# MCG-NJU/MeMOTR

Measured on AMD Instinct MI355X. Metric: train_frames_per_sec, higher is better.
Workload: dtype f32

## Files before the change

### memotr_amd/csrc/clip_attention.h

```cpp
#pragma once

namespace {
constexpr int kLanes = 16;
constexpr int kRows = 256 / kLanes;
constexpr int kHd = 32;
constexpr int kPitch = 36;

__device__ __forceinline__ void load_row32(const float *p, float *r) {
#pragma unroll
    for (int i = 0; i < 8; ++i) {
        const f32x4_t v = *reinterpret_cast<const f32x4_t *>(p + 4 * i);
        r[4 * i] = v.x; r[4 * i + 1] = v.y; r[4 * i + 2] = v.z; r[4 * i + 3] = v.w;
    }
}

__device__ __forceinline__ float dot32(const float *a, const float *lds_row) {
    float s0 = 0.f, s1 = 0.f;
#pragma unroll
    for (int i = 0; i < 8; ++i) {
        const f32x4_t v = *reinterpret_cast<const f32x4_t *>(lds_row + 4 * i);
        s0 = fmaf(a[4 * i], v.x, s0);
        s1 = fmaf(a[4 * i + 1], v.y, s1);
        s0 = fmaf(a[4 * i + 2], v.z, s0);
        s1 = fmaf(a[4 * i + 3], v.w, s1);
    }
    return s0 + s1;
}

__device__ __forceinline__ float dot32r(const float *a, const float *b) {
    float s0 = 0.f, s1 = 0.f;
#pragma unroll
    for (int i = 0; i < 8; ++i) {
        s0 = fmaf(a[4 * i], b[4 * i], s0);
        s1 = fmaf(a[4 * i + 1], b[4 * i + 1], s1);
        s0 = fmaf(a[4 * i + 2], b[4 * i + 2], s0);
        s1 = fmaf(a[4 * i + 3], b[4 * i + 3], s1);
    }
    return s0 + s1;
}

__device__ __forceinline__ void axpy32(float *acc, float w, const float *lds_row) {
#pragma unroll
    for (int i = 0; i < 8; ++i) {
        const f32x4_t v = *reinterpret_cast<const f32x4_t *>(lds_row + 4 * i);
        acc[4 * i] = fmaf(w, v.x, acc[4 * i]);
        acc[4 * i + 1] = fmaf(w, v.y, acc[4 * i + 1]);
        acc[4 * i + 2] = fmaf(w, v.z, acc[4 * i + 2]);
        acc[4 * i + 3] = fmaf(w, v.w, acc[4 * i + 3]);
    }
}

__device__ __forceinline__ float sum8l(float x) {
#pragma unroll
    for (int o = 1; o < kLanes; o <<= 1) x += __shfl_xor(x, o, 64);
    return x;
}
__device__ __forceinline__ float max8l(float x) {
#pragma unroll
    for (int o = 1; o < kLanes; o <<= 1) x = fmaxf(x, __shfl_xor(x, o, 64));
    return x;
}

__device__ __forceinline__ void stage_rows(float *dst, const float *src, long rs, int L) {
    for (int i = threadIdx.x; i < L * 8; i += blockDim.x) {
        const int r = i >> 3, c = (i & 7) * 4;
        *reinterpret_cast<f32x4_t *>(dst + r * kPitch + c) = *reinterpret_cast<const f32x4_t *>(src + r * rs + c);
    }
}

__global__ __launch_bounds__(256) void mha_fwd_kernel(const float *__restrict__ q, const float *__restrict__ k,
                                                     const float *__restrict__ v, long q_bs, long q_rs, long k_bs,
                                                     long k_rs, long v_bs, long v_rs,
                                                     const uint8_t *__restrict__ key_mask, int H, int L, float scale,
                                                     float *__restrict__ out, float *__restrict__ lse) {
    extern __shared__ __attribute__((aligned(16))) float s_mem[];
    float *Ks = s_mem, *Vs = s_mem + (size_t)L * kPitch;
    const int h = blockIdx.y, b = blockIdx.z;
    stage_rows(Ks, k + b * k_bs + h * kHd, k_rs, L);
    stage_rows(Vs, v + b * v_bs + h * kHd, v_rs, L);
    __syncthreads();
    const int row = blockIdx.x * kRows + threadIdx.x / kLanes, sub = threadIdx.x % kLanes;
    const bool row_ok = row < L;
    const int rowc = row_ok ? row : L - 1;
    float qr[kHd];
    load_row32(q + b * q_bs + rowc * q_rs + h * kHd, qr);
#pragma unroll
    for (int i = 0; i < kHd; ++i) qr[i] *= scale;
    const uint8_t *mk = key_mask ? key_mask + (long)b * L : nullptr;
    float m = -INFINITY, l = 0.f, acc[kHd];
#pragma unroll
    for (int i = 0; i < kHd; ++i) acc[i] = 0.f;
    for (int j = sub; j < L; j += kLanes) {
        if (mk && mk[j]) continue;
        const float s = dot32(qr, Ks + j * kPitch);
        const float m_new = fmaxf(m, s);
        const float corr = expf(m - m_new), p = expf(s - m_new);
        l = l * corr + p;
#pragma unroll
        for (int i = 0; i < kHd; ++i) acc[i] *= corr;
        axpy32(acc, p, Vs + j * kPitch);
        m = m_new;
    }
    const float M = max8l(m);
    const float w = (m == -INFINITY) ? 0.f : expf(m - M);
    const float Lsum = sum8l(l * w);
    const float inv = 1.f / Lsum;
    float *o = out + ((long)b * L + rowc) * (H * kHd) + h * kHd;
#pragma unroll
    for (int i = 0; i < kHd; ++i) {
        const float t = sum8l(acc[i] * w) * inv;
        if (row_ok && (i >> 2) == sub) o[i] = t;
    }
    if (row_ok && sub == 0) lse[((long)b * H + h) * L + row] = M + logf(Lsum);
}

__global__ __launch_bounds__(256) void mha_bwd_q_kernel(const float *__restrict__ q, const float *__restrict__ k,
                                                       const float *__restrict__ v, long q_bs, long q_rs, long k_bs,
                                                       long k_rs, long v_bs, long v_rs,
                                                       const uint8_t *__restrict__ key_mask,
                                                       const float *__restrict__ out, const float *__restrict__ lse,
                                                       const float *__restrict__ go, int H, int L, float scale,
                                                       float *__restrict__ gq, long gq_bs, long gq_rs) {
    extern __shared__ __attribute__((aligned(16))) float s_mem[];
    float *Ks = s_mem, *Vs = s_mem + (size_t)L * kPitch;
    const int h = blockIdx.y, b = blockIdx.z;
    stage_rows(Ks, k + b * k_bs + h * kHd, k_rs, L);
    stage_rows(Vs, v + b * v_bs + h * kHd, v_rs, L);
    __syncthreads();
    const int row = blockIdx.x * kRows + threadIdx.x / kLanes, sub = threadIdx.x % kLanes;
    const bool row_ok = row < L;
    const int rowc = row_ok ? row : L - 1;
    float qr[kHd], gr[kHd], acc[kHd];
    load_row32(q + b * q_bs + rowc * q_rs + h * kHd, qr);
    const long orow = ((long)b * L + rowc) * (H * kHd) + h * kHd;
    load_row32(go + orow, gr);
    float D = 0.f;
    {
        float orr[kHd];
        load_row32(out + orow, orr);
        D = dot32r(gr, orr);
    }
#pragma unroll
    for (int i = 0; i < kHd; ++i) { qr[i] *= scale; acc[i] = 0.f; }
    const float ls = lse[((long)b * H + h) * L + rowc];
    const uint8_t *mk = key_mask ? key_mask + (long)b * L : nullptr;
    for (int j = sub; j < L; j += kLanes) {
        if (mk && mk[j]) continue;
        const float p = expf(dot32(qr, Ks + j * kPitch) - ls);
        const float ds = p * (dot32(gr, Vs + j * kPitch) - D);
        axpy32(acc, ds, Ks + j * kPitch);
    }
    float *g = gq + b * gq_bs + rowc * gq_rs + h * kHd;
#pragma unroll
    for (int i = 0; i < kHd; ++i) {
        const float t = sum8l(acc[i]) * scale;
        if (row_ok && (i >> 2) == sub) g[i] = t;
    }
}

__global__ __launch_bounds__(256) void mha_bwd_kv_kernel(const float *__restrict__ q, const float *__restrict__ k,
                                                        const float *__restrict__ v, long q_bs, long q_rs, long k_bs,
                                                        long k_rs, long v_bs, long v_rs,
                                                        const uint8_t *__restrict__ key_mask,
                                                        const float *__restrict__ out, const float *__restrict__ lse,
                                                        const float *__restrict__ go, int H, int L, float scale,
                                                        float *__restrict__ gk, long gk_bs, long gk_rs,
                                                        float *__restrict__ gv, long gv_bs, long gv_rs) {
    extern __shared__ __attribute__((aligned(16))) float s_mem[];
    float *Qs = s_mem, *Gs = s_mem + (size_t)L * kPitch;
    float *s_lse = Gs + (size_t)L * kPitch, *s_D = s_lse + L;
    const int h = blockIdx.y, b = blockIdx.z;
    stage_rows(Qs, q + b * q_bs + h * kHd, q_rs, L);
    for (int i = threadIdx.x; i < L * 8; i += blockDim.x) {
        f32x4_t *p4 = reinterpret_cast<f32x4_t *>(Qs + (i >> 3) * kPitch + (i & 7) * 4);
        *p4 = *p4 * scale;
    }
    stage_rows(Gs, go + (long)b * L * (H * kHd) + h * kHd, (long)H * kHd, L);
    for (int i = threadIdx.x; i < L; i += blockDim.x) s_lse[i] = lse[((long)b * H + h) * L + i];
    __syncthreads();
    for (int i = threadIdx.x; i < L; i += blockDim.x) {
        const float *o = out + ((long)b * L + i) * (H * kHd) + h * kHd;
        float orr[kHd];
        load_row32(o, orr);
        s_D[i] = dot32(orr, Gs + i * kPitch);
    }
    __syncthreads();
    const int row = blockIdx.x * kRows + threadIdx.x / kLanes, sub = threadIdx.x % kLanes;
    const bool row_ok = row < L;
    const int rowc = row_ok ? row : L - 1;
    const bool dead = key_mask && key_mask[(long)b * L + rowc];
    float kr[kHd], vr[kHd], ak[kHd], av[kHd];
    load_row32(k + b * k_bs + rowc * k_rs + h * kHd, kr);
    load_row32(v + b * v_bs + rowc * v_rs + h * kHd, vr);
#pragma unroll
    for (int i = 0; i < kHd; ++i) { ak[i] = 0.f; av[i] = 0.f; }
    if (!dead) {
        for (int i = sub; i < L; i += kLanes) {
            const float p = expf(dot32(kr, Qs + i * kPitch) - s_lse[i]);
            const float ds = p * (dot32(vr, Gs + i * kPitch) - s_D[i]);
            axpy32(av, p, Gs + i * kPitch);
            axpy32(ak, ds, Qs + i * kPitch);
        }
    }
    float *pk = gk + b * gk_bs + rowc * gk_rs + h * kHd, *pv = gv + b * gv_bs + rowc * gv_rs + h * kHd;
#pragma unroll
    for (int i = 0; i < kHd; ++i) {
        const float tk = sum8l(ak[i]), tv = sum8l(av[i]);
        if (row_ok && (i >> 2) == sub) {
            pk[i] = tk;
            pv[i] = tv;
        }
    }
}

std::atomic<unsigned long long> g_lds_fwd{0}, g_lds_bq{0}, g_lds_bkv{0};

int mha_check(const void *q, const void *k, const void *v, int B, int H, int L) {
    if (B < 0 || H <= 0 || L < 0) return fail(1, "clipops_mha: bad dimension");
    if (L > CLIPOPS_MHA_MAX_L) return fail(2, "clipops_mha: L exceeds CLIPOPS_MHA_MAX_L");
    if ((long)B * L > 0 && (!q || !k || !v)) return fail(1, "clipops_mha: null pointer");
    return 0;
}
}

extern "C" {
int clipops_mha_fwd_f32(const float *q, const float *k, const float *v, long q_bs, long q_rs, long k_bs, long k_rs,
                        long v_bs, long v_rs, const uint8_t *key_mask, int B, int H, int L, float scale, float *out,
                        float *lse, void *stream) {
    int rc = mha_check(q, k, v, B, H, L);
    if (rc) return rc;
    if ((long)B * L == 0) return ok();
    if (!out || !lse) return fail(1, "clipops_mha_fwd_f32: null pointer");
    const size_t lds = (size_t)2 * L * kPitch * sizeof(float);
    if ((rc = allow_lds(reinterpret_cast<const void *>(mha_fwd_kernel), lds, g_lds_fwd))) return rc;
    return launch("mha_fwd_kernel", mha_fwd_kernel, dim3((L + kRows - 1) / kRows, H, B), dim3(256), lds, stream, q, k, v,
                  q_bs, q_rs, k_bs, k_rs, v_bs, v_rs, key_mask, H, L, scale, out, lse);
}

int clipops_mha_bwd_f32(const float *q, const float *k, const float *v, long q_bs, long q_rs, long k_bs, long k_rs,
                        long v_bs, long v_rs, const uint8_t *key_mask, const float *out, const float *lse,
                        const float *grad_out, int B, int H, int L, float scale, float *grad_q, long gq_bs, long gq_rs,
                        float *grad_k, long gk_bs, long gk_rs, float *grad_v, long gv_bs, long gv_rs, void *stream) {
    int rc = mha_check(q, k, v, B, H, L);
    if (rc) return rc;
    if ((long)B * L == 0) return ok();
    if (!out || !lse || !grad_out || !grad_q || !grad_k || !grad_v) return fail(1, "clipops_mha_bwd_f32: null pointer");
    const size_t lds_q = (size_t)2 * L * kPitch * sizeof(float);
    const size_t lds_kv = lds_q + (size_t)2 * L * sizeof(float);
    if ((rc = allow_lds(reinterpret_cast<const void *>(mha_bwd_q_kernel), lds_q, g_lds_bq))) return rc;
    if ((rc = allow_lds(reinterpret_cast<const void *>(mha_bwd_kv_kernel), lds_kv, g_lds_bkv))) return rc;
    const dim3 grid((L + kRows - 1) / kRows, H, B);
    if ((rc = launch("mha_bwd_q_kernel", mha_bwd_q_kernel, grid, dim3(256), lds_q, stream, q, k, v, q_bs, q_rs, k_bs, k_rs,
                     v_bs, v_rs, key_mask, out, lse, grad_out, H, L, scale, grad_q, gq_bs, gq_rs)))
        return rc;
    return launch("mha_bwd_kv_kernel", mha_bwd_kv_kernel, grid, dim3(256), lds_kv, stream, q, k, v, q_bs, q_rs, k_bs, k_rs,
                  v_bs, v_rs, key_mask, out, lse, grad_out, H, L, scale, grad_k, gk_bs, gk_rs, grad_v, gv_bs, gv_rs);
}
}
```

### memotr_amd/functions/clip_ops.py

```python
from __future__ import annotations

import ctypes
import os

import torch
import torch.nn.functional as F


def fused(*tensors) -> bool:
    return (os.environ.get("MEMOTR_FUSED_CLIP_OPS", "1") != "0"
            and all(t.is_cuda and (t.dtype == torch.float32 or not t.is_floating_point()) for t in tensors))


def config_key() -> tuple:
    return (os.environ.get("MEMOTR_FUSED_CLIP_OPS", "1"), os.environ.get("MEMOTR_COLSUM_TALL", "1"),
            os.environ.get("MEMOTR_ATTN_KERNELS", "1"), os.environ.get("MEMOTR_FUSED_LN", "1"),
            os.environ.get("MEMOTR_FUSED_SHIFT_RELU", "1"), os.environ.get("MEMOTR_FUSED_LINEAR_BWD", "1"),
            os.environ.get("MEMOTR_FUSED_LINEAR_FWD", "1"), os.environ.get("MEMOTR_LINEAR_STAGED", "1"))


def _lib():
    from .. import _clip_lib
    return _clip_lib


def _stream(t: torch.Tensor) -> int:
    idx = t.device.index
    if idx is not None and idx != torch.cuda.current_device():
        raise RuntimeError(f"clip_ops: tensor on cuda:{idx} but cuda:{torch.cuda.current_device()} is current; "
                           "call torch.cuda.set_device(tensor.device) (one device per process)")
    return torch.cuda.current_stream(t.device).cuda_stream


def _strides3(t: torch.Tensor):
    if t.dim() != 3 or (t.shape[2] > 1 and t.stride(2) != 1):
        raise RuntimeError("expected a (layers, rows, C) tensor with a dense last axis")
    return t.stride(0), t.stride(1)


def match_cost(logits: torch.Tensor, boxes: torch.Tensor, gt_labels: torch.Tensor, gt_boxes: torch.Tensor,
               w_class: float, w_bbox: float, w_giou: float, out: torch.Tensor = None) -> torch.Tensor:
    n_layers, Q, K = logits.shape
    T = gt_labels.shape[0]
    if out is not None:
        assert out.is_contiguous() and out.dtype == torch.float32 and out.numel() == n_layers * Q * T
        cost = out.view(n_layers, Q, T)
    else:
        cost = torch.empty((n_layers, Q, T), dtype=torch.float32, device=logits.device)
    lsl, lsq = _strides3(logits)
    bsl, bsq = _strides3(boxes)
    gt_labels, gt_boxes = gt_labels.contiguous(), gt_boxes.contiguous()
    L = _lib()
    L.check(L.lib.clipops_match_cost_f32(logits.data_ptr(), lsl, lsq, boxes.data_ptr(), bsl, bsq, gt_labels.data_ptr(),
                                         gt_boxes.data_ptr(), n_layers, Q, K, T, float(w_class), float(w_bbox),
                                         float(w_giou), cost.data_ptr(), _stream(logits)), "clipops_match_cost_f32")
    return cost


def track_ownership(track_ids: torch.Tensor, gt_ids: torch.Tensor, free_out: torch.Tensor = None):
    n_tr, n_gt = track_ids.shape[0], gt_ids.shape[0]
    matched = torch.empty((n_tr,), dtype=torch.int64, device=gt_ids.device)
    free = free_out if free_out is not None else torch.empty((n_gt,), dtype=torch.float32, device=gt_ids.device)
    assert free.is_contiguous() and free.dtype == torch.float32 and free.numel() == n_gt
    track_ids, gt_ids = track_ids.contiguous(), gt_ids.contiguous()
    L = _lib()
    L.check(L.lib.clipops_track_ownership_i64(track_ids.data_ptr(), n_tr, gt_ids.data_ptr(), n_gt, matched.data_ptr(),
                                              free.data_ptr(), _stream(gt_ids)), "clipops_track_ownership_i64")
    return matched, free


def track_ownership_reference(track_ids, gt_ids):
    n_gt = gt_ids.shape[0]
    eq = track_ids[:, None] == gt_ids[None, :]
    order = torch.arange(1, n_gt + 1, device=eq.device)
    return (eq * order).amax(1) - 1 if n_gt > 0 else torch.full_like(track_ids, -1), (~eq.any(0)).to(torch.float32)


def focal_labels(lay: torch.Tensor, q: torch.Tensor, g: torch.Tensor, gt_labels: torch.Tensor, matched_idx,
                 late: torch.Tensor, n_det: int, n_tracks: int, num_classes: int) -> torch.Tensor:
    n_layers = late.shape[0]
    labels = torch.empty((n_layers, n_det + n_tracks), dtype=torch.int64, device=late.device)
    lay, q, g, gt_labels = lay.contiguous(), q.contiguous(), g.contiguous(), gt_labels.contiguous()
    L = _lib()
    L.check(L.lib.clipops_focal_labels_i64(lay.data_ptr(), q.data_ptr(), g.data_ptr(), lay.shape[0], gt_labels.data_ptr(),
                                           gt_labels.shape[0], None if matched_idx is None else matched_idx.contiguous().data_ptr(),
                                           n_tracks, late.contiguous().data_ptr(), n_layers, n_det, num_classes,
                                           labels.data_ptr(), _stream(late)), "clipops_focal_labels_i64")
    return labels


def focal_labels_reference(lay, q, g, gt_labels, matched_idx, late, n_det, n_tracks, num_classes):
    n_layers = late.shape[0]
    labels = torch.full((n_layers, n_det + n_tracks), num_classes, dtype=torch.int64, device=late.device)
    labels[lay, q] = gt_labels[g]
    if n_tracks > 0:
        has = matched_idx >= 0
        tr_lab = torch.where(has, gt_labels[matched_idx.clamp(min=0)] if gt_labels.shape[0] > 0
                             else torch.full_like(matched_idx, num_classes), torch.full_like(matched_idx, num_classes))
        labels[:, n_det:] = torch.where(late[:, None], tr_lab[None, :], labels[:, n_det:])
    return labels


class _PairBoxLoss(torch.autograd.Function):
    @staticmethod
    def forward(ctx, boxes_all, lay, qidx, b, tgt_boxes, gidx, weight):
        n_layers, B, Nq, _ = boxes_all.shape
        n = lay.shape[0]
        l1 = torch.empty((n,), dtype=torch.float32, device=boxes_all.device)
        gl = torch.empty_like(l1)
        L = _lib()
        L.check(L.lib.clipops_pair_box_loss_fwd_f32(
            boxes_all.data_ptr(), lay.data_ptr(), qidx.data_ptr(), B * Nq, b * Nq, tgt_boxes.data_ptr(),
            None if gidx is None else gidx.data_ptr(), None if weight is None else weight.data_ptr(), n,
            l1.data_ptr(), gl.data_ptr(), _stream(boxes_all)), "clipops_pair_box_loss_fwd_f32")
        ctx.save_for_backward(boxes_all, lay, qidx, tgt_boxes, gidx, weight)
        ctx.b = b
        return l1, gl

    @staticmethod
    def backward(ctx, g_l1, g_gl):
        boxes_all, lay, qidx, tgt_boxes, gidx, weight = ctx.saved_tensors
        n_layers, B, Nq, _ = boxes_all.shape
        grad = torch.zeros_like(boxes_all)
        L = _lib()
        L.check(L.lib.clipops_pair_box_loss_bwd_f32(
            boxes_all.data_ptr(), lay.data_ptr(), qidx.data_ptr(), B * Nq, ctx.b * Nq, tgt_boxes.data_ptr(),
            None if gidx is None else gidx.data_ptr(), None if weight is None else weight.data_ptr(), lay.shape[0],
            g_l1.contiguous().data_ptr(), g_gl.contiguous().data_ptr(), grad.data_ptr(), _stream(boxes_all)),
            "clipops_pair_box_loss_bwd_f32")
        return grad, None, None, None, None, None, None


def pair_box_loss(boxes_all: torch.Tensor, lay: torch.Tensor, qidx: torch.Tensor, b: int, tgt_boxes: torch.Tensor,
                  gidx: torch.Tensor = None, weight: torch.Tensor = None):
    if not boxes_all.is_contiguous():
        boxes_all = boxes_all.contiguous()
    return _PairBoxLoss.apply(boxes_all, lay.contiguous(), qidx.contiguous(), int(b), tgt_boxes.contiguous(),
                              None if gidx is None else gidx.contiguous(),
                              None if weight is None else weight.contiguous())


def pair_box_loss_reference(boxes_all, lay, qidx, b, tgt_boxes, gidx=None, weight=None):
    from ..models.criterion import paired_giou
    from ..utils.box_ops import box_cxcywh_to_xyxy
    pb = boxes_all[lay, b, qidx]
    tb = tgt_boxes if gidx is None else tgt_boxes[gidx]
    l1 = F.l1_loss(pb, tb, reduction="none").sum(-1)
    gl = 1 - paired_giou(box_cxcywh_to_xyxy(pb), box_cxcywh_to_xyxy(tb))
    if weight is not None:
        l1, gl = l1 * weight, gl * weight
    return l1, gl


def pair_iou(boxes: torch.Tensor, tgt_boxes: torch.Tensor, gidx: torch.Tensor = None) -> torch.Tensor:
    boxes, tgt_boxes = boxes.detach().contiguous(), tgt_boxes.contiguous()
    n = boxes.shape[0]
    out = torch.empty((n,), dtype=torch.float32, device=boxes.device)
    L = _lib()
    L.check(L.lib.clipops_pair_iou_f32(boxes.data_ptr(), tgt_boxes.data_ptr(), None if gidx is None else
                                       gidx.contiguous().data_ptr(), n, out.data_ptr(), _stream(boxes)),
            "clipops_pair_iou_f32")
    return out


def assign(cost: torch.Tensor):
    if cost.dim() != 3 or cost.dtype != torch.float32 or not cost.is_cuda:
        raise RuntimeError("assign expects a float32 CUDA tensor of shape (problems, rows, cols)")
    P, R, C = cost.shape
    k = min(R, C)
    row = torch.empty((P, k), dtype=torch.int32, device=cost.device)
    col = torch.empty((P, k), dtype=torch.int32, device=cost.device)
    status = torch.empty((P,), dtype=torch.int32, device=cost.device)
    L = _lib()
    L.check(L.lib.clipops_assign_f32(cost.data_ptr(), cost.stride(0), cost.stride(1), cost.stride(2), P, R, C,
                                     row.data_ptr(), col.data_ptr(), status.data_ptr(), _stream(cost)),
            "clipops_assign_f32")
    return row, col, status


def pair_iou_reference(boxes, tgt_boxes, gidx=None):
    from ..models.criterion import paired_iou
    from ..utils.box_ops import box_cxcywh_to_xyxy
    tb = tgt_boxes if gidx is None else tgt_boxes[gidx]
    return paired_iou(box_cxcywh_to_xyxy(boxes), box_cxcywh_to_xyxy(tb))


HANDOVER_CARRIED, HANDOVER_NEW, HANDOVER_UNCLAIMED = 0, 1, 2
HANDOVER_DIFF = ("outputs", "queries", "last_ref", "init_ref", "det_embed", "prev_ref", "prev_long", "prev_last",
                 "prev_query")


def handover_tables(n_det: int, n_q: int, n_tracks: int, new_q, new_g, free_q, keep):
    import numpy as np
    n_new, n_free = len(new_q), len(free_q)
    kind = np.concatenate((np.full((n_tracks,), HANDOVER_CARRIED, dtype=np.int64),
                           np.full((n_new,), HANDOVER_NEW, dtype=np.int64),
                           np.full((n_free,), HANDOVER_UNCLAIMED, dtype=np.int64)))
    src = np.concatenate((np.arange(n_tracks, dtype=np.int64), np.asarray(new_q, dtype=np.int64),
                          np.asarray(free_q, dtype=np.int64)))
    gt = np.concatenate((np.full((n_tracks,), -1, dtype=np.int64), np.asarray(new_g, dtype=np.int64),
                         np.full((n_free,), -1, dtype=np.int64)))
    keep = np.asarray(keep, dtype=np.int64)
    table = np.stack((kind[keep], src[keep], gt[keep]), axis=1)
    rows = np.arange(len(keep), dtype=np.int64)
    carried = table[:, 0] == HANDOVER_CARRIED
    inv_q = np.full((n_q,), -1, dtype=np.int64)
    inv_q[np.where(carried, n_det + table[:, 1], table[:, 1])] = rows
    inv_prev = np.full((n_tracks,), -1, dtype=np.int64)
    inv_prev[table[carried, 1]] = rows[carried]
    return np.concatenate((table.reshape(-1), inv_q, inv_prev))


def _handover_views(tables, n_keep, n_q, n_tracks):
    table = tables[:3 * n_keep]
    inv_q = tables[3 * n_keep:3 * n_keep + n_q]
    inv_prev = tables[3 * n_keep + n_q:3 * n_keep + n_q + n_tracks]
    return table, inv_q, inv_prev


def _rows_dense(t):
    return t if t.dim() == 2 and (t.shape[1] == 1 or t.stride(1) == 1) and t.stride(0) >= 0 else t.contiguous()


class _Handover(torch.autograd.Function):
    @staticmethod
    def forward(ctx, outputs, queries, last_ref, init_ref, det_embed, prev_ref, prev_long, prev_last, prev_query,
                logits, boxes, prev_iou, prev_ids, prev_matched, gt_boxes, gt_ids, tables, n_keep, n_det):
        L = _lib()
        use_dab = det_embed is None
        n_q, C, K = outputs.shape[0], outputs.shape[1], logits.shape[1]
        n_tracks, n_gt = prev_ref.shape[0], gt_boxes.shape[0]
        QW = C if use_dab else 2 * C
        named = dict(logits=logits, boxes=boxes, outputs=outputs, queries=queries, last_ref=last_ref, init_ref=init_ref,
                     det_embed=det_embed, prev_ref=prev_ref, prev_long=prev_long, prev_last=prev_last,
                     prev_query=prev_query, prev_iou=prev_iou.reshape(-1, 1))
        widths = dict(logits=K, boxes=4, outputs=C, queries=C, last_ref=4, init_ref=4, det_embed=C, prev_ref=4,
                      prev_long=C, prev_last=C, prev_query=QW, prev_iou=1)
        src, keep = L.HandoverSources(), []
        for i, name in enumerate(L.HANDOVER_SOURCES):
            t = named[name]
            if t is None or t.shape[0] == 0:
                continue
            lead = n_tracks if name.startswith("prev_") else (n_det if name == "det_embed" else n_det + n_tracks)
            if t.dtype != torch.float32 or t.dim() != 2 or t.shape[0] < lead or (
                    t.shape[1] != widths[name] and not (name == "det_embed" and t.shape[1] >= C)):
                raise RuntimeError(f"handover: source {name} has shape {tuple(t.shape)} ({t.dtype})")
            t = _rows_dense(t.detach())
            keep.append(t)
            src.ptr[i], src.row_stride[i] = t.data_ptr(), t.stride(0)
        if n_q != queries.shape[0] or n_q != last_ref.shape[0] or n_q != init_ref.shape[0]:
            raise RuntimeError("handover: the model-output sources differ in their row counts")
        if tables.dtype != torch.int64 or tables.numel() != 3 * n_keep + n_q + n_tracks:
            raise RuntimeError("handover: the table does not have 3 * n_keep + n_q + n_tracks int64 entries")
        tables = tables.contiguous()
        prev_ids, prev_matched, gt_boxes, gt_ids = (t.contiguous() for t in (prev_ids, prev_matched, gt_boxes, gt_ids))
        if n_tracks and (prev_ids.shape[0] != n_tracks or prev_matched.shape[0] != n_tracks):
            raise RuntimeError("handover: ids / matched_idx of the previous set do not have one entry per track")
        dev = outputs.device
        base = torch.empty((n_keep, K + 8 + 3 * C + QW + 1), dtype=torch.float32, device=dev)
        ints = torch.empty((2, n_keep), dtype=torch.int64, device=dev)
        L.check(L.lib.clipops_handover_fwd_f32(
            ctypes.byref(src), prev_ids.data_ptr() if n_tracks else None, prev_matched.data_ptr() if n_tracks else None,
            gt_boxes.data_ptr(), gt_ids.data_ptr(), tables.data_ptr(), n_keep, n_det, n_tracks, n_gt, K, C,
            int(use_dab), base.data_ptr(), ints[0].data_ptr(), ints[1].data_ptr(), _stream(outputs)),
            "clipops_handover_fwd_f32")
        ctx.save_for_backward(tables)
        ctx.dims = (n_keep, n_q, n_det, n_tracks, K, C, use_dab, 0 if det_embed is None else det_embed.shape[1], QW)
        ctx.mark_non_differentiable(ints)
        return base, ints

    @staticmethod
    def backward(ctx, g_base, _g_ints):
        L = _lib()
        (tables,) = ctx.saved_tensors
        n_keep, n_q, n_det, n_tracks, K, C, use_dab, det_cols, QW = ctx.dims
        table, inv_q, inv_prev = _handover_views(tables, n_keep, n_q, n_tracks)
        g_base = g_base.contiguous()
        shapes = dict(outputs=(n_q, C), queries=(n_q, C), last_ref=(n_q, 4), init_ref=(n_q, 4),
                      det_embed=(n_det, det_cols), prev_ref=(n_tracks, 4), prev_long=(n_tracks, C),
                      prev_last=(n_tracks, C), prev_query=(n_tracks, QW))
        wanted = [name for i, name in enumerate(HANDOVER_DIFF) if ctx.needs_input_grad[i]]
        flat = torch.empty((sum(shapes[n][0] * shapes[n][1] for n in wanted),), dtype=torch.float32, device=g_base.device)
        grads, out, pos = L.HandoverGrads(), {}, 0
        for name in wanted:
            r, c = shapes[name]
            out[name] = flat[pos:pos + r * c].view(r, c)
            pos += r * c
            if r * c:
                grads.ptr[L.HANDOVER_SOURCES.index(name)] = out[name].data_ptr()
        if flat.numel():
            L.check(L.lib.clipops_handover_bwd_f32(
                g_base.data_ptr(), table.data_ptr(), inv_q.data_ptr(), inv_prev.data_ptr() if n_tracks else None,
                n_keep, n_q, n_det, n_tracks, K, C, int(use_dab), det_cols, ctypes.byref(grads), _stream(g_base)),
                "clipops_handover_bwd_f32")
        return tuple(out.get(name) for name in HANDOVER_DIFF) + (None,) * 10


def handover(outputs, queries, last_ref, init_ref, det_embed, prev_ref, prev_long, prev_last, prev_query, logits, boxes,
             prev_iou, prev_ids, prev_matched, gt_boxes, gt_ids, tables, n_keep: int, n_det: int):
    base, ints = _Handover.apply(outputs, queries, last_ref, init_ref, det_embed, prev_ref, prev_long, prev_last,
                                 prev_query, logits, boxes, prev_iou, prev_ids, prev_matched, gt_boxes, gt_ids, tables,
                                 n_keep, n_det)
    return base, ints[0], ints[1]


def handover_reference(outputs, queries, last_ref, init_ref, det_embed, prev_ref, prev_long, prev_last, prev_query,
                       logits, boxes, prev_iou, prev_ids, prev_matched, gt_boxes, gt_ids, tables, n_keep: int,
                       n_det: int):
    n_q, C = outputs.shape
    n_tracks = prev_ref.shape[0]
    table, _, _ = _handover_views(tables, n_keep, n_q, n_tracks)
    kind, s, g = table.view(n_keep, 3).unbind(1)
    carried, new = (kind == HANDOVER_CARRIED), (kind == HANDOVER_NEW)
    m = torch.where(carried, n_det + s, s)
    q = torch.where(carried, torch.zeros_like(s), s)

    def prev(t):
        width = 1 if t.dim() == 1 else t.shape[1]
        if n_tracks == 0:
            return t.new_zeros((n_keep, width))
        return t.reshape(n_tracks, width)[torch.where(carried, s, torch.zeros_like(s))]
# ... 742 lines not shown
```

Baseline: 43.67.

## Add v2 fused attention kernels with wider rows, DPP reductions, merged backward

Adds new forward and backward MHA kernels enabled by default via MEMOTR_MHA_V2. The forward kernel uses 512-thread blocks with 32 lanes per query row and caches scores in LDS for a two-pass softmax. It reuses one LDS buffer for K then V (prefetched into registers), skips masked keys, and reduces across lanes with DPP and swizzle. The backward pass merges the dQ and dK/dV kernels into one launch that splits blocks by index and skips dead keys. This cuts launch count and shuffle cost, but adds register pressure and LDS footprint and relies on CLIPOPS_MHA_MAX_L bounds.

```diff
diff --git a/memotr_amd/csrc/clip_attention.h b/memotr_amd/csrc/clip_attention.h
--- a/memotr_amd/csrc/clip_attention.h
+++ b/memotr_amd/csrc/clip_attention.h
@@ -213,7 +213,229 @@
     }
 }
 
-std::atomic<unsigned long long> g_lds_fwd{0}, g_lds_bq{0}, g_lds_bkv{0};
+#define MHA_DPP(x, ctrl) \
+    __builtin_bit_cast(float, __builtin_amdgcn_update_dpp(0, __builtin_bit_cast(int, (x)), (ctrl), 0xF, 0xF, true))
+
+template <int LANES>
+__device__ __forceinline__ float row_sum(float x) {
+    x += MHA_DPP(x, 0xB1);
+    x += MHA_DPP(x, 0x4E);
+    x += MHA_DPP(x, 0x141);
+    x += MHA_DPP(x, 0x140);
+    if (LANES == 32) x += __builtin_bit_cast(float, __builtin_amdgcn_ds_swizzle(__builtin_bit_cast(int, x), 0x401F));
+    return x;
+}
+template <int LANES>
+__device__ __forceinline__ float row_max(float x) {
+    x = fmaxf(x, MHA_DPP(x, 0xB1));
+    x = fmaxf(x, MHA_DPP(x, 0x4E));
+    x = fmaxf(x, MHA_DPP(x, 0x141));
+    x = fmaxf(x, MHA_DPP(x, 0x140));
+    if (LANES == 32) x = fmaxf(x, __builtin_bit_cast(float, __builtin_amdgcn_ds_swizzle(__builtin_bit_cast(int, x), 0x401F)));
+    return x;
+}
+
+constexpr int kLanesW = 32;
+constexpr int kRowsW = 512 / kLanesW;
+constexpr int kRowsQ = 512 / kLanes;
+
+template <int LANES>
+__device__ __forceinline__ unsigned live_keys(const uint8_t *s_mk, int sub, int L) {
+    unsigned live = 0;
+    for (int t = 0; t * LANES < L; ++t) {
+        const int j = sub + t * LANES;
+        const bool on = j < L && !(s_mk && s_mk[min(j, L - 1)]);
+        live |= (unsigned)on << t;
+    }
+    return live;
+}
+
+__host__ __device__ inline size_t mask_bytes(int L) { return (size_t)(L + 15) / 16 * 16; }
+
+__global__ __launch_bounds__(512) void mha2_fwd_kernel(const float *__restrict__ q, const float *__restrict__ k,
+                                                      const float *__restrict__ v, long q_bs, long q_rs, long k_bs,
+                                                      long k_rs, long v_bs, long v_rs,
+                                                      const uint8_t *__restrict__ key_mask, int H, int L, float scale,
+                                                      float *__restrict__ out, float *__restrict__ lse) {
+    constexpr int NV = CLIPOPS_MHA_MAX_L * 8 / 512;
+    extern __shared__ __attribute__((aligned(16))) float s_mem[];
+    const int n_t = (L + kLanesW - 1) / kLanesW;
+    float *s_sc = s_mem + (size_t)L * kPitch + threadIdx.x;
+    uint8_t *s_mk = reinterpret_cast<uint8_t *>(s_mem + (size_t)L * kPitch + (size_t)n_t * 512);
+    const int h = blockIdx.y, b = blockIdx.z;
+    const float *kp = k + b * k_bs + h * kHd, *vp = v + b * v_bs + h * kHd;
+    f32x4_t kreg[NV], vreg[NV];
+#pragma unroll
+    for (int t = 0; t < NV; ++t) {
+        const int i = threadIdx.x + t * 512;
+        if (i < L * 8) kreg[t] = *reinterpret_cast<const f32x4_t *>(kp + (i >> 3) * k_rs + (i & 7) * 4);
+    }
+#pragma unroll
+    for (int t = 0; t < NV; ++t) {
+        const int i = threadIdx.x + t * 512;
+        if (i < L * 8) vreg[t] = *reinterpret_cast<const f32x4_t *>(vp + (i >> 3) * v_rs + (i & 7) * 4);
+    }
+    if (key_mask && (int)threadIdx.x < L) s_mk[threadIdx.x] = key_mask[(long)b * L + threadIdx.x];
+    const int row = blockIdx.x * kRowsW + threadIdx.x / kLanesW, sub = threadIdx.x % kLanesW;
+    const bool row_ok = row < L;
+    const int rowc = row_ok ? row : L - 1;
+    float qr[kHd];
+    load_row32(q + b * q_bs + rowc * q_rs + h * kHd, qr);
+#pragma unroll
+    for (int i = 0; i < kHd; ++i) qr[i] *= scale;
+#pragma unroll
+    for (int t = 0; t < NV; ++t) {
+        const int i = threadIdx.x + t * 512;
+        if (i < L * 8) *reinterpret_cast<f32x4_t *>(s_mem + (i >> 3) * kPitch + (i & 7) * 4) = kreg[t];
+    }
+    __syncthreads();
+    const unsigned live = live_keys<kLanesW>(key_mask ? s_mk : nullptr, sub, L);
+    float m = -INFINITY;
+#pragma unroll 4
+    for (int t = 0; t < n_t; ++t) {
+        const int jc = min(sub + t * kLanesW, L - 1);
+        const float s = (live >> t) & 1u ? dot32(qr, s_mem + jc * kPitch) : -INFINITY;
+        s_sc[t * 512] = s;
+        m = fmaxf(m, s);
+    }
+    const float M = row_max<kLanesW>(m);
+    __syncthreads();
+#pragma unroll
+    for (int t = 0; t < NV; ++t) {
+        const int i = threadIdx.x + t * 512;
+        if (i < L * 8) *reinterpret_cast<f32x4_t *>(s_mem + (i >> 3) * kPitch + (i & 7) * 4) = vreg[t];
+    }
+    __syncthreads();
+    float l = 0.f, acc[kHd];
+#pragma unroll
+    for (int i = 0; i < kHd; ++i) acc[i] = 0.f;
+#pragma unroll 2
+    for (int t = 0; t < n_t; ++t) {
+        const int jc = min(sub + t * kLanesW, L - 1);
+        const float p = (live >> t) & 1u ? expf(s_sc[t * 512] - M) : 0.f;
+        l += p;
+        axpy32(acc, p, s_mem + jc * kPitch);
+    }
+    const float Lsum = row_sum<kLanesW>(l);
+    const float inv = 1.f / Lsum;
+    float *o = out + ((long)b * L + rowc) * (H * kHd) + h * kHd;
+#pragma unroll
+    for (int i = 0; i < kHd; ++i) {
+        const float t = row_sum<kLanesW>(acc[i]) * inv;
+        if (row_ok && (i >> 2) == sub) o[i] = t;
+    }
+    if (row_ok && sub == 0) lse[((long)b * H + h) * L + row] = M + logf(Lsum);
+}
+
+__global__ __launch_bounds__(512) void mha2_bwd_kernel(const float *__restrict__ q, const float *__restrict__ k,
+                                                      const float *__restrict__ v, long q_bs, long q_rs, long k_bs,
+                                                      long k_rs, long v_bs, long v_rs,
+                                                      const uint8_t *__restrict__ key_mask,
+                                                      const float *__restrict__ out, const float *__restrict__ lse,
+                                                      const float *__restrict__ go, int H, int L, float scale,
+                                                      float *__restrict__ gq, long gq_bs, long gq_rs,
+                                                      float *__restrict__ gk, long gk_bs, long gk_rs,
+                                                      float *__restrict__ gv, long gv_bs, long gv_rs, int nblk_q) {
+    extern __shared__ __attribute__((aligned(16))) float s_mem[];
+    float *As = s_mem, *Bs = s_mem + (size_t)L * kPitch;
+    float *s_lse = Bs + (size_t)L * kPitch, *s_D = s_lse + L;
+    const int h = blockIdx.y, b = blockIdx.z;
+    const long orow0 = (long)b * L * (H * kHd) + h * kHd;
+    if ((int)blockIdx.x < nblk_q) {
+        uint8_t *s_mk = reinterpret_cast<uint8_t *>(s_D + L);
+        const int row = blockIdx.x * kRowsQ + threadIdx.x / kLanes, sub = threadIdx.x % kLanes;
+        const bool row_ok = row < L;
+        const int rowc = row_ok ? row : L - 1;
+        float qr[kHd], gr[kHd], acc[kHd];
+        load_row32(q + b * q_bs + rowc * q_rs + h * kHd, qr);
+        load_row32(go + orow0 + (long)rowc * (H * kHd), gr);
+        float D;
+        {
+            float orr[kHd];
+            load_row32(out + orow0 + (long)rowc * (H * kHd), orr);
+            D = dot32r(gr, orr);
+        }
+#pragma unroll
+        for (int i = 0; i < kHd; ++i) { qr[i] *= scale; acc[i] = 0.f; }
+        const float ls = lse[((long)b * H + h) * L + rowc];
+        if (key_mask && (int)threadIdx.x < L) s_mk[threadIdx.x] = key_mask[(long)b * L + threadIdx.x];
+        stage_rows(As, k + b * k_bs + h * kHd, k_rs, L);
+        stage_rows(Bs, v + b * v_bs + h * kHd, v_rs, L);
+        __syncthreads();
+        const unsigned live = live_keys<kLanes>(key_mask ? s_mk : nullptr, sub, L);
+        for (int t = 0; t * kLanes < L; ++t) {
+            const int jc = min(sub + t * kLanes, L - 1);
+            const bool on = (live >> t) & 1u;
+            const float p = expf(dot32(qr, As + jc * kPitch) - ls);
+            const float ds = on ? p * (dot32(gr, Bs + jc * kPitch) - D) : 0.f;
+            axpy32(acc, ds, As + jc * kPitch);
+        }
+        float *g = gq + b * gq_bs + rowc * gq_rs + h * kHd;
+#pragma unroll
+        for (int i = 0; i < kHd; ++i) {
+            const float t = row_sum<kLanes>(acc[i]) * scale;
+            if (row_ok && (i >> 2) == sub) g[i] = t;
+        }
+        return;
+    }
+    const int row = (blockIdx.x - nblk_q) * kRowsW + threadIdx.x / kLanesW, sub = threadIdx.x % kLanesW;
+    const bool row_ok = row < L;
+    const int rowc = row_ok ? row : L - 1;
+    f32x4_t qreg[8];
+    const float *qp = q + b * q_bs + h * kHd;
+#pragma unroll
+    for (int t = 0; t < 8; ++t) {
+        const int i = threadIdx.x + t * 512;
+        if (i < L * 8) qreg[t] = *reinterpret_cast<const f32x4_t *>(qp + (i >> 3) * q_rs + (i & 7) * 4) * scale;
+    }
+    const bool dead = key_mask && key_mask[(long)b * L + rowc];
+    float kr[kHd], vr[kHd], ak[kHd], av[kHd];
+    load_row32(k + b * k_bs + rowc * k_rs + h * kHd, kr);
+    load_row32(v + b * v_bs + rowc * v_rs + h * kHd, vr);
+    stage_rows(As, out + orow0, (long)H * kHd, L);
+    stage_rows(Bs, go + orow0, (long)H * kHd, L);
+    for (int i = threadIdx.x; i < L; i += blockDim.x) s_lse[i] = lse[((long)b * H + h) * L + i];
+    __syncthreads();
+    for (int i = threadIdx.x; i < L; i += blockDim.x) {
+        float orr[kHd];
+        load_row32(As + i * kPitch, orr);
+        s_D[i] = dot32(orr, Bs + i * kPitch);
+    }
+    __syncthreads();
+#pragma unroll
+    for (int t = 0; t < 8; ++t) {
+        const int i = threadIdx.x + t * 512;
+        if (i < L * 8) *reinterpret_cast<f32x4_t *>(As + (i >> 3) * kPitch + (i & 7) * 4) = qreg[t];
+    }
+    __syncthreads();
+#pragma unroll
+    for (int i = 0; i < kHd; ++i) { ak[i] = 0.f; av[i] = 0.f; }
+    if (!dead) {
+        for (int t = 0; t * kLanesW < L; ++t) {
+            const int i = sub + t * kLanesW, ic = min(i, L - 1);
+            const float p = i < L ? expf(dot32(kr, As + ic * kPitch) - s_lse[ic]) : 0.f;
+            const float ds = p * (dot32(vr, Bs + ic * kPitch) - s_D[ic]);
+            axpy32(av, p, Bs + ic * kPitch);
+            axpy32(ak, ds, As + ic * kPitch);
+        }
+    }
+    float *pk = gk + b * gk_bs + rowc * gk_rs + h * kHd, *pv = gv + b * gv_bs + rowc * gv_rs + h * kHd;
+#pragma unroll
+    for (int i = 0; i < kHd; ++i) {
+        const float tk = row_sum<kLanesW>(ak[i]), tv = row_sum<kLanesW>(av[i]);
+        if (row_ok && (i >> 2) == sub) {
+            pk[i] = tk;
+            pv[i] = tv;
+        }
+    }
+}
+
+bool mha_v2() {
+    const char *e = getenv("MEMOTR_MHA_V2");
+    return !(e && e[0] == '0' && e[1] == 0);
+}
+
+std::atomic<unsigned long long> g_lds_fwd{0}, g_lds_bq{0}, g_lds_bkv{0}, g_lds_fwd2{0}, g_lds_bwd2{0};
 
 int mha_check(const void *q, const void *k, const void *v, int B, int H, int L) {
     if (B < 0 || H <= 0 || L < 0) return fail(1, "clipops_mha: bad dimension");
@@ -231,6 +453,12 @@
     if (rc) return rc;
     if ((long)B * L == 0) return ok();
     if (!out || !lse) return fail(1, "clipops_mha_fwd_f32: null pointer");
+    if (mha_v2()) {
+        const size_t lds = ((size_t)L * kPitch + (size_t)((L + kLanesW - 1) / kLanesW) * 512) * sizeof(float) + mask_bytes(L);
+        if ((rc = allow_lds(reinterpret_cast<const void *>(mha2_fwd_kernel), lds, g_lds_fwd2))) return rc;
+        return launch("mha2_fwd_kernel", mha2_fwd_kernel, dim3((L + kRowsW - 1) / kRowsW, H, B), dim3(512), lds, stream, q,
+                      k, v, q_bs, q_rs, k_bs, k_rs, v_bs, v_rs, key_mask, H, L, scale, out, lse);
+    }
     const size_t lds = (size_t)2 * L * kPitch * sizeof(float);
     if ((rc = allow_lds(reinterpret_cast<const void *>(mha_fwd_kernel), lds, g_lds_fwd))) return rc;
     return launch("mha_fwd_kernel", mha_fwd_kernel, dim3((L + kRows - 1) / kRows, H, B), dim3(256), lds, stream, q, k, v,
@@ -247,6 +475,14 @@
     if (!out || !lse || !grad_out || !grad_q || !grad_k || !grad_v) return fail(1, "clipops_mha_bwd_f32: null pointer");
     const size_t lds_q = (size_t)2 * L * kPitch * sizeof(float);
     const size_t lds_kv = lds_q + (size_t)2 * L * sizeof(float);
+    if (mha_v2()) {
+        const size_t lds = lds_kv + mask_bytes(L);
+        if ((rc = allow_lds(reinterpret_cast<const void *>(mha2_bwd_kernel), lds, g_lds_bwd2))) return rc;
+        const int nblk_q = (L + kRowsQ - 1) / kRowsQ, nblk_kv = (L + kRowsW - 1) / kRowsW;
+        return launch("mha2_bwd_kernel", mha2_bwd_kernel, dim3(nblk_q + nblk_kv, H, B), dim3(512), lds, stream, q, k, v,
+                      q_bs, q_rs, k_bs, k_rs, v_bs, v_rs, key_mask, out, lse, grad_out, H, L, scale, grad_q, gq_bs, gq_rs,
+                      grad_k, gk_bs, gk_rs, grad_v, gv_bs, gv_rs, nblk_q);
+    }
     if ((rc = allow_lds(reinterpret_cast<const void *>(mha_bwd_q_kernel), lds_q, g_lds_bq))) return rc;
     if ((rc = allow_lds(reinterpret_cast<const void *>(mha_bwd_kv_kernel), lds_kv, g_lds_bkv))) return rc;
     const dim3 grid((L + kRows - 1) / kRows, H, B);
diff --git a/memotr_amd/functions/clip_ops.py b/memotr_amd/functions/clip_ops.py
--- a/memotr_amd/functions/clip_ops.py
+++ b/memotr_amd/functions/clip_ops.py
@@ -16,7 +16,8 @@
     return (os.environ.get("MEMOTR_FUSED_CLIP_OPS", "1"), os.environ.get("MEMOTR_COLSUM_TALL", "1"),
             os.environ.get("MEMOTR_ATTN_KERNELS", "1"), os.environ.get("MEMOTR_FUSED_LN", "1"),
             os.environ.get("MEMOTR_FUSED_SHIFT_RELU", "1"), os.environ.get("MEMOTR_FUSED_LINEAR_BWD", "1"),
-            os.environ.get("MEMOTR_FUSED_LINEAR_FWD", "1"), os.environ.get("MEMOTR_LINEAR_STAGED", "1"))
+            os.environ.get("MEMOTR_FUSED_LINEAR_FWD", "1"), os.environ.get("MEMOTR_LINEAR_STAGED", "1"),
+            os.environ.get("MEMOTR_MHA_V2", "1"))
 
 
 def _lib():
```

Result: no change. 44.21, median of 6 (+1.2%).
